# lim0606/pytorch-ardae-vae

Hardware: AMD Instinct MI355X
Metric: AR-DAE-VAE train-steps/sec (batch 512, nz_cdae 256) on dbMNIST (higher is better)
Workload: dtype f32

## Files before the change

### include/ardae_hip.h

```cpp
#ifndef ARDAE_HIP_H
#define ARDAE_HIP_H

#include <stddef.h>
#include <stdint.h>

#ifdef __cplusplus
extern "C" {
#endif

#define ARDAE_ABI_VERSION 1

enum { ARDAE_ACT_NONE = 0, ARDAE_ACT_RELU = 1, ARDAE_ACT_SOFTPLUS = 2, ARDAE_ACT_ELU = 3, ARDAE_ACT_TANH = 4, ARDAE_ACT_LEAKY_RELU = 5, ARDAE_ACT_SWISH = 6 };

enum {
  ARDAE_EPI_ACT = 0,
  ARDAE_EPI_DACT = 1,
  ARDAE_EPI_CHAIN = 2,
  ARDAE_EPI_DAE_LOSS = 3
};

typedef struct ardae_lin_src {
  const float* x;
  int ld;
  int K;
// ... 15 lines not shown
  const float* R; int ldR;
  const float* Q; int ldQ;
  const float* sigma;
  const float* eps; int ldeps;
  float scale;
  float* Y;  int ldY;
  float* Y2; int ldY2;
  float* colsum;
  float* tile_loss;
} ardae_linear_args;

const char* ardae_last_error(void);
int ardae_abi_version(void);

size_t ardae_packed_floats(int nout, int k);
int ardae_linear_row_tiles(int M, int nout);
int ardae_linear_col_panels(int M, int nout);
int ardae_pack_weight(const float* W, int ldw, int nout, int k, int transpose, float* out, void* stream);
int ardae_linear(const ardae_linear_args* args, int epilogue, void* stream);
int ardae_linear_chain_eligible(const ardae_linear_args* layers, int nl, int epilogue);
int ardae_linear_chain(const ardae_linear_args* layers, int nl, int epilogue, void* stream);
int ardae_linear_wide_layers_eligible(const ardae_linear_args* layers, int nl, int epilogue);
int ardae_linear_wide_layers(const ardae_linear_args* layers, int nl, int epilogue, void* stream);


#define ARDAE_WGRAD_MAX_PROBLEMS 20
typedef struct ardae_wgrad_problem {
  int M, O, I;
  int npairs;
  const float* G[2]; int ldG[2];
  const float* X[2]; int ldX[2];
  int bias_pair;
  const float* rowscale;
  int splits;
  float* partial;
  float* partial_vec;
  float* out; int ldout;
  float* out_bias;
  float* out_rowscale; int ld_rowscale;
  float beta;
} ardae_wgrad_problem;
int ardae_wgrad_splits(int M, int O, int I, int nproblems_hint);
int ardae_wgrad_batch(const ardae_wgrad_problem* problems, int nproblems, void* stream);


int ardae_latent_perturb(const float* latent, const float* z0, const float* xi, const float* eps, int B, int nz, int z,
// ... 133 lines not shown
```

### pytorch-ardae-vae_amd/_lib.py

```python
import ctypes
import os

_HERE = os.path.dirname(os.path.abspath(__file__))
LIB_PATH = os.environ.get("ARDAE_LIB") or os.path.join(_HERE, "libardae_hip.so")

c_float_p = ctypes.POINTER(ctypes.c_float)


def debug_knob(name, default=None):
    if os.environ.get("ARDAE_DEBUG_KNOBS") != "1":
        return default
    return os.environ.get(name, default)


class LinSrc(ctypes.Structure):
    _fields_ = [("x", ctypes.c_void_p), ("ld", ctypes.c_int), ("K", ctypes.c_int), ("wp", ctypes.c_void_p)]


class LinearArgs(ctypes.Structure):
    _fields_ = [
        ("M", ctypes.c_int), ("Nout", ctypes.c_int),
        ("nsrc", ctypes.c_int),
        ("src", LinSrc * 2),
        ("act", ctypes.c_int),
# ... 49 lines not shown
MODEL_HEAD_SHIFT = 1
MODEL_CLIPPED = 16
LOGVAR_CLIP = {None: 0, "none": 0, "hard": 1, "softplus": 2, "spm10": 3, "spm6": 4, "spm5": 5, "spm4": 6, "spm3": 7, "spm2": 8, "tanh": 9, "2tanh": 10}
MODEL_CLIP_Z0_SHIFT, MODEL_CLIP_Z_SHIFT = 8, 12


ACT = {"none": 0, None: 0, "relu": 1, "softplus": 2, "csoftplus": 2, "elu": 3, "tanh": 4, "leaky_relu": 5, "swish": 6}
LOG_RECORD_FLOATS = 16
EPI_ACT, EPI_DACT, EPI_CHAIN, EPI_DAE_LOSS = 0, 1, 2, 3

EXPORTS = {
    "ardae_last_error": (ctypes.c_char_p, []),
    "ardae_abi_version": (ctypes.c_int, []),
    "ardae_packed_floats": (ctypes.c_size_t, [ctypes.c_int, ctypes.c_int]),
    "ardae_linear_row_tiles": (ctypes.c_int, [ctypes.c_int, ctypes.c_int]),
    "ardae_linear_col_panels": (ctypes.c_int, [ctypes.c_int, ctypes.c_int]),
    "ardae_pack_weight": (ctypes.c_int, [ctypes.c_void_p, ctypes.c_int, ctypes.c_int, ctypes.c_int, ctypes.c_int,
                                         ctypes.c_void_p, ctypes.c_void_p]),
    "ardae_linear": (ctypes.c_int, [ctypes.POINTER(LinearArgs), ctypes.c_int, ctypes.c_void_p]),
    "ardae_linear_chain_eligible": (ctypes.c_int, [ctypes.POINTER(LinearArgs), ctypes.c_int, ctypes.c_int]),
    "ardae_linear_chain": (ctypes.c_int, [ctypes.POINTER(LinearArgs), ctypes.c_int, ctypes.c_int, ctypes.c_void_p]),
    "ardae_linear_wide_layers_eligible": (ctypes.c_int, [ctypes.POINTER(LinearArgs), ctypes.c_int, ctypes.c_int]),
    "ardae_linear_wide_layers": (ctypes.c_int, [ctypes.POINTER(LinearArgs), ctypes.c_int, ctypes.c_int, ctypes.c_void_p]),
    "ardae_wgrad_splits": (ctypes.c_int, [ctypes.c_int] * 4),
    "ardae_wgrad_batch": (ctypes.c_int, [ctypes.POINTER(WgradProblem), ctypes.c_int, ctypes.c_void_p]),
    "ardae_latent_perturb": (ctypes.c_int, [ctypes.c_void_p] * 4 + [ctypes.c_int] * 3 + [ctypes.c_float] * 2 + [ctypes.c_void_p] * 4),
    "ardae_latent_perturb_nstd": (ctypes.c_int, [ctypes.c_void_p] * 4 + [ctypes.c_int] * 4 + [ctypes.c_float] * 2 + [ctypes.c_void_p] * 4),
    "ardae_latent_perturb_draw_ok": (ctypes.c_int, [ctypes.c_int] * 3),
    "ardae_latent_perturb_draw": (ctypes.c_int, [ctypes.c_void_p] * 2 + [ctypes.c_int] * 3 + [ctypes.c_float] * 2 + [ctypes.c_uint64] * 3 +
                                  [ctypes.c_void_p, ctypes.c_uint64] + [ctypes.c_void_p] * 5),
    "ardae_cdae_perturb_fused_ok": (ctypes.c_int, [ctypes.c_void_p, ctypes.c_int, ctypes.c_int]),
    "ardae_cdae_perturb_loss_grads": (ctypes.c_int, [ctypes.c_void_p] * 6 + [ctypes.c_int] * 2 + [ctypes.c_float] * 2 + [ctypes.c_uint64] * 3 +
                                      [ctypes.c_void_p, ctypes.c_uint64] + [ctypes.c_void_p] * 5 + [ctypes.c_size_t] + [ctypes.c_void_p] * 3),
    "ardae_center_scale": (ctypes.c_int, [ctypes.c_void_p] * 2 + [ctypes.c_int] * 3 + [ctypes.c_float] + [ctypes.c_void_p] * 2),
    "ardae_philox_normal": (ctypes.c_int, [ctypes.c_void_p, ctypes.c_int64, ctypes.c_uint64, ctypes.c_uint64, ctypes.c_void_p]),
    "ardae_philox_uniform": (ctypes.c_int, [ctypes.c_void_p, ctypes.c_int64, ctypes.c_uint64, ctypes.c_uint64, ctypes.c_void_p]),
    "ardae_bernoulli": (ctypes.c_int, [ctypes.c_void_p, ctypes.c_int64, ctypes.c_int, ctypes.c_void_p, ctypes.c_uint64,
                                       ctypes.c_uint64, ctypes.c_void_p]),
    "ardae_step_state_advance": (ctypes.c_int, [ctypes.c_void_p, ctypes.c_uint64, ctypes.c_double, ctypes.c_double, ctypes.c_double, ctypes.c_void_p]),
    "ardae_philox_normal_dev": (ctypes.c_int, [ctypes.c_void_p, ctypes.c_int64, ctypes.c_uint64, ctypes.c_void_p, ctypes.c_uint64, ctypes.c_void_p]),
    "ardae_philox_normal_at": (ctypes.c_int, [ctypes.c_void_p, ctypes.c_int64, ctypes.c_uint64, ctypes.c_uint64, ctypes.c_void_p, ctypes.c_uint64,
                                               ctypes.c_void_p]),
    "ardae_adam_ref_step_dev": (ctypes.c_int, [ctypes.c_void_p] * 5 + [ctypes.c_int64] + [ctypes.c_double] * 3 + [ctypes.c_void_p, ctypes.c_void_p]),
    "ardae_adam_ref_step": (ctypes.c_int, [ctypes.c_void_p] * 5 + [ctypes.c_int64] + [ctypes.c_double] * 4 + [ctypes.c_int, ctypes.c_void_p]),
    "ardae_weight_avg": (ctypes.c_int, [ctypes.c_void_p] * 2 + [ctypes.c_int64, ctypes.c_int, ctypes.c_double, ctypes.c_int64, ctypes.c_void_p,
                                         ctypes.c_int64, ctypes.c_void_p]),
# ... 102 lines not shown
```

### pytorch-ardae-vae_amd/csrc/api.hip

```cpp
#include <stdarg.h>

#include "ardae_hip.h"
#include "common.h"
#include "elementwise.h"
#include "linear.h"
#include "wgrad.h"

namespace ardae {
static thread_local char g_last_error[512] = "";
void set_last_error(const char* fmt, ...) {
  va_list ap;
  va_start(ap, fmt);
  vsnprintf(g_last_error, sizeof(g_last_error), fmt, ap);
  va_end(ap);
}
}

using namespace ardae;

extern "C" {

const char* ardae_last_error(void) { return g_last_error; }
int ardae_abi_version(void) { return ARDAE_ABI_VERSION; }

size_t ardae_packed_floats(int nout, int k) { return packed_floats(nout, k); }
int ardae_linear_row_tiles(int M, int nout) { return linear_row_tiles(M, nout); }
int ardae_linear_col_panels(int M, int nout) { return linear_col_panels(M, nout); }

int ardae_pack_weight(const float* W, int ldw, int nout, int k, int transpose, float* out, void* stream) {
  return launch_pack_weight(W, ldw, nout, k, transpose != 0, out, (hipStream_t)stream);
}

int ardae_linear(const ardae_linear_args* args, int epilogue, void* stream) {
  ARDAE_CHECK_ARG(args != nullptr, "ardae_linear: args is NULL");
  return launch_linear(*args, epilogue, (hipStream_t)stream);
}

int ardae_linear_wide_layers_eligible(const ardae_linear_args* layers, int nl, int epilogue) {
  return layers && linear_wide_layers_eligible(layers, nl, epilogue) ? 1 : 0;
}
int ardae_linear_wide_layers(const ardae_linear_args* layers, int nl, int epilogue, void* stream) {
  ARDAE_CHECK_ARG(layers != nullptr, "ardae_linear_wide_layers: layers is NULL");
  return launch_linear_wide_layers(layers, nl, epilogue, (hipStream_t)stream);
}
int ardae_linear_chain_eligible(const ardae_linear_args* layers, int nl, int epilogue) {
  return (layers != nullptr && linear_chain_eligible(layers, nl, epilogue)) ? 1 : 0;
}
int ardae_linear_chain(const ardae_linear_args* layers, int nl, int epilogue, void* stream) {
  ARDAE_CHECK_ARG(layers != nullptr, "ardae_linear_chain: layers is NULL");
  return launch_linear_chain(layers, nl, epilogue, (hipStream_t)stream);
}

int ardae_wgrad_splits(int M, int O, int I, int nproblems_hint) { return wgrad_splits(M, O, I, nproblems_hint); }
int ardae_wgrad_batch(const ardae_wgrad_problem* problems, int nproblems, void* stream) {
  return launch_wgrad_batch(problems, nproblems, (hipStream_t)stream);
}

int ardae_latent_perturb(const float* latent, const float* z0, const float* xi, const float* eps, int B, int nz, int z,
                         float std_scale, float delta, float* xbar, float* sigma, float* std_b, void* stream) {
  return launch_latent_perturb(latent, z0, xi, eps, B, nz, 1, z, std_scale, delta, xbar, sigma, std_b, (hipStream_t)stream);
}
int ardae_latent_perturb_nstd(const float* latent, const float* z0, const float* xi, const float* eps, int B, int nz, int nstd, int z,
                              float std_scale, float delta, float* xbar, float* sigma, float* std_b, void* stream) {
  return launch_latent_perturb(latent, z0, xi, eps, B, nz, nstd, z, std_scale, delta, xbar, sigma, std_b, (hipStream_t)stream);
}
int ardae_latent_perturb_draw_ok(int nz, int nstd, int z) { return latent_perturb_draw_ok(nz, nstd, z) ? 1 : 0; }
// ... 49 lines not shown
```

### pytorch-ardae-vae_amd/csrc/cdae.hip

```cpp
#include <vector>

#include "ardae_hip.h"
#include "common.h"
#include "elementwise.h"
#include "linear.h"
#include "wgrad.h"

namespace ardae {
namespace {

#define PACK_PUSH(W_, ldw_, nout_, k_, tr_, out_) pack_items__.push_back(PackItem{W_, ldw_, nout_, k_, (tr_) ? 1 : 0, out_})
#define PACK_FLUSH(st_) ARDAE_TRY(launch_pack_batch(pack_items__.data(), (int)pack_items__.size(), st_))

struct Lin {
  size_t w, b;
  int out, in;
};

struct CdaeLayout {
  int kind, z, c, h, L, act;
  std::vector<Lin> ctx, inp, neg;
  size_t total = 0;
  int out_dim() const { return kind == 0 ? 1 : z; }

// ... 118 lines not shown
    PACK_PUSH(params + P.neg[l].w, P.h, P.h, P.h, false, packed + K.neg_f[l]);
    PACK_PUSH(params + P.neg[l].w, P.h, P.h, P.h, true, packed + K.neg_b[l]);
  }
  if (P.kind == 1) {
    PACK_PUSH(params + P.neg[P.L].w, P.h, P.z, P.h, false, packed + K.fc_f);
    PACK_PUSH(params + P.neg[P.L].w, P.h, P.h, P.z, true, packed + K.fc_b);
  }
  PACK_FLUSH(st);
  return 0;
}

LinArgs lin_args(int act, int M, int Nout, const float* x, int ldx, int K, const float* wp, LinArgs a) {
  a.M = M; a.Nout = Nout; a.nsrc = 1; a.act = act;
  a.src[0].x = x; a.src[0].ld = ldx; a.src[0].K = K; a.src[0].wp = wp;
  return a;
}
int lin(int epi, int act, int M, int Nout, const float* x, int ldx, int K, const float* wp, LinArgs a, hipStream_t st) {
  return launch_linear(lin_args(act, M, Nout, x, ldx, K, wp, a), epi, st);
}

struct LayerRun {
  int epi;
  hipStream_t st;
  std::vector<LinArgs> v;
  LayerRun(int epi_, hipStream_t st_) : epi(epi_), st(st_) {}
  void add(int act, int M, int Nout, const float* x, int ldx, int K, const float* wp, LinArgs a) { v.push_back(lin_args(act, M, Nout, x, ldx, K, wp, a)); }
  int flush() {
    size_t i = 0;
    while (i < v.size()) {
      size_t n = v.size() - i;
      while (n >= 2 && !linear_chain_eligible(v.data() + i, (int)n, epi)) --n;
      if (n >= 2) {
        ARDAE_TRY(launch_linear_chain(v.data() + i, (int)n, epi, st));
        i += n;
        continue;
      }
      size_t m = std::min<size_t>(v.size() - i, 6);
      while (m >= 2 && !linear_wide_layers_eligible(v.data() + i, (int)m, epi)) --m;
      if (m >= 2) {
        ARDAE_TRY(launch_linear_wide_layers(v.data() + i, (int)m, epi, st));
        i += m;
      } else {
        ARDAE_TRY(launch_linear(v[i], epi, st));
        i += 1;
      }
    }
    v.clear();
    return 0;
  }
};

float* cdae_a1_slot(const CdaeLayout& P, int B, float* workspace) {
  Bump ws(workspace, ~size_t(0));
  for (int l = 0; l <= P.L; ++l) ws.take((size_t)B * P.h);
  return ws.take(1);
}

int cdae_impl(const ardae_cdae_desc* d, const float* params, const float* packed, const float* xbar, const float* sigma,
              const float* eps, const float* ctx, int B, int S, float* workspace, size_t ws_floats, float* loss, float* grads,
              float* score_out, bool need_grads, hipStream_t st, bool a1_ready = false) {
  ARDAE_TRY(desc_ok(d));
  ARDAE_CHECK_ARG(params && packed && xbar && sigma && ctx && workspace, "cdae: null pointer argument");
  ARDAE_CHECK_ARG(B > 0 && S > 0 && (int64_t)B * S < (int64_t)1 << 30, "cdae: bad batch (B=%d, S=%d)", B, S);
  ARDAE_CHECK_ARG(!need_grads || (eps && loss && grads), "cdae: loss/grads/eps must be given");
  ARDAE_CHECK_ARG(need_grads || score_out, "cdae: score_out is NULL");
  const CdaeLayout P(*d);
  const PackedLayout K(P);
  const int N = B * S, h = P.h, L = P.L, z = P.z, act = P.act;
  ARDAE_CHECK_ARG(ws_floats >= workspace_floats(P, B, S, need_grads), "cdae: workspace too small (%zu < %zu floats)", ws_floats,
                  workspace_floats(P, B, S, need_grads));
// ... 22 lines not shown
    std::vector<LinArgs> pr; std::vector<int> ep, lv;
    int level = 0;
    auto add = [&](const LinArgs& A, int epi, int lev) { pr.push_back(A); ep.push_back(epi); lv.push_back(lev); };
    for (int l = 1; l <= L; ++l, ++level) { add(ctx_layer(l), EPI_ACT, level); add(inp_layer(l), EPI_ACT, level); }
    { LinArgs A{}; A.bias = params + P.neg[0].b; A.Y = cb; A.ldY = h; add(lin_args(ACT_NONE, B, h, cL[L], h, h, packed + K.w1c_f, A), EPI_ACT, level++); }
    for (int l = 1; l <= L; ++l) {
      LinArgs A{}; A.Y = hh[l]; A.ldY = h;
      if (l == 1) { A.rowbias = cb; A.rowbias_ld = h; A.rows_per_group = S; A.rowscale = sigma; A.rowscale_w = W1s; } else A.bias = params + P.neg[l - 1].b;
      if (l == L) { A.Y2 = e[L]; A.ldY2 = h; A.R = wfc0; }
      add(lin_args(act, N, h, l == 1 ? a[L] : hh[l - 1], h, h, l == 1 ? packed + K.w1a_f : packed + K.neg_f[l - 1], A), EPI_ACT, level++);
    }
    for (int l = L; l >= 2; --l) { LinArgs A{}; A.S = hh[l - 1]; A.ldS = h; A.Y = e[l - 1]; A.ldY = h; add(lin_args(act, N, h, e[l], h, h, packed + K.neg_b[l - 1], A), EPI_DACT, level++); }
    { LinArgs A{}; A.S = a[L]; A.ldS = h; A.Y = r[L]; A.ldY = h; add(lin_args(act, N, h, e[1], h, h, packed + K.w1a_b, A), EPI_DACT, level++); }
    for (int l = L; l >= 2; --l) { LinArgs A{}; A.S = a[l - 1]; A.ldS = h; A.Y = r[l - 1]; A.ldY = h; add(lin_args(act, N, h, r[l], h, h, packed + K.inp_b[l - 1], A), EPI_DACT, level++); }
    { LinArgs A{}; A.Y = g; A.ldY = z; add(lin_args(ACT_NONE, N, z, r[1], h, h, packed + K.inp_b[0], A), EPI_ACT, level++); }
    return launch_linear_small_chain(pr.data(), ep.data(), lv.data(), (int)pr.size(), chain_cnt, st);
  }
  ARDAE_CHECK_ARG(!a1_ready || a[1] == cdae_a1_slot(P, B, workspace), "cdae: a_1 slot moved (workspace layout and cdae_a1_slot disagree)");
  const bool few_rows = !a1_ready && linear_small_eligible(inp_layer(1), EPI_ACT);
  auto ctx_bias = [&]() {
    LinArgs A{}; A.bias = params + P.neg[0].b; A.Y = cb; A.ldY = h;
    return lin(EPI_ACT, ACT_NONE, B, h, cL[L], h, h, packed + K.w1c_f, A, st);
  };
  LayerRun run(EPI_ACT, st);
  if (few_rows) {
    for (int l = 1; l <= L; ++l) ARDAE_TRY(launch_linear_pair(ctx_layer(l), inp_layer(l), EPI_ACT, st));
    ARDAE_TRY(ctx_bias());
  } else {
    for (int l = 1; l <= L; ++l) ARDAE_TRY(launch_linear(ctx_layer(l), EPI_ACT, st));
    ARDAE_TRY(ctx_bias());
    for (int l = a1_ready ? 2 : 1; l <= L; ++l) run.v.push_back(inp_layer(l));
  }
  const float* wfc = params + P.neg[L].w;
  {
    for (int l = 1; l <= L; ++l) {
      LinArgs A{}; A.Y = hh[l]; A.ldY = h;
      if (l == 1) {
        A.rowbias = cb; A.rowbias_ld = h; A.rows_per_group = S; A.rowscale = sigma; A.rowscale_w = W1s;
      } else {
        A.bias = params + P.neg[l - 1].b;
      }
      if (P.kind == 0 && l == L) { A.Y2 = e[L]; A.ldY2 = h; A.R = wfc; }
      run.add(act, N, h, l == 1 ? a[L] : hh[l - 1], h, h, l == 1 ? packed + K.w1a_f : packed + K.neg_f[l - 1], A);
    }
    ARDAE_TRY(run.flush());
  }
  const float inv_nz = 1.0f / ((float)N * (float)z);
  if (P.kind == 0) {
    {
      LayerRun run(EPI_DACT, st);
      for (int l = L; l >= 2; --l) {
        LinArgs A{}; A.S = hh[l - 1]; A.ldS = h; A.Y = e[l - 1]; A.ldY = h;
        run.add(act, N, h, e[l], h, h, packed + K.neg_b[l - 1], A);
      }
      {
        LinArgs A{}; A.S = a[L]; A.ldS = h; A.Y = r[L]; A.ldY = h;
        run.add(act, N, h, e[1], h, h, packed + K.w1a_b, A);
      }
      for (int l = L; l >= 2; --l) {
        LinArgs A{}; A.S = a[l - 1]; A.ldS = h; A.Y = r[l - 1]; A.ldY = h;
        run.add(act, N, h, r[l], h, h, packed + K.inp_b[l - 1], A);
      }
      ARDAE_TRY(run.flush());
    }
    if (!need_grads) {
      LinArgs A{}; A.Y = g; A.ldY = z;
      return lin(EPI_ACT, ACT_NONE, N, z, r[1], h, h, packed + K.inp_b[0], A, st);
    }
    LinArgs A{}; A.sigma = sigma; A.eps = eps; A.ldeps = z; A.scale = inv_nz; A.Y = g; A.ldY = z; A.Y2 = gbar; A.ldY2 = z;
    A.tile_loss = tile_loss;
    ARDAE_TRY(lin(EPI_DAE_LOSS, ACT_NONE, N, z, r[1], h, h, packed + K.inp_b[0], A, st));
  } else {
    if (!need_grads) {
      LinArgs A{}; A.bias = params + P.neg[L].b; A.Y = g; A.ldY = z;
      return lin(EPI_ACT, ACT_NONE, N, z, hh[L], h, h, packed + K.fc_f, A, st);
    }
    LinArgs A{}; A.bias = params + P.neg[L].b; A.sigma = sigma; A.eps = eps; A.ldeps = z; A.scale = inv_nz; A.Y = g; A.ldY = z;
    A.Y2 = gbar; A.ldY2 = z; A.tile_loss = tile_loss;
    ARDAE_TRY(lin(EPI_DAE_LOSS, ACT_NONE, N, z, hh[L], h, h, packed + K.fc_f, A, st));
  }
  ARDAE_TRY(launch_sum_scale(tile_loss, ltiles, inv_nz, loss, st));

  float* Qsum = ws.take(Bh);
  for (int l = 1; l <= L; ++l) chat[l] = ws.take(Bh);
  const int ctiles = linear_row_tiles(N, h);
  float* cs_taup = ws.take((size_t)ctiles * h);
  std::vector<float*>&qhat = qbar, &phat = pbar;
  if (P.kind == 0) {
    {
      LayerRun run(EPI_CHAIN, st);
      for (int l = 1; l <= L; ++l) {
        LinArgs A{}; A.S = a[l]; A.ldS = h; A.R = r[l]; A.ldR = h; A.Y = tau[l]; A.ldY = h; A.Y2 = pbar[l]; A.ldY2 = h;
        if (l == 1) run.add(act, N, h, gbar, z, z, packed + K.inp_f[0], A);
        else run.add(act, N, h, tau[l - 1], h, h, packed + K.inp_f[l - 1], A);
      }
      for (int l = 1; l <= L; ++l) {
        LinArgs A{}; A.S = hh[l]; A.ldS = h; A.R = e[l]; A.ldR = h; A.Y = taup[l]; A.ldY = h; A.Y2 = qbar[l]; A.ldY2 = h;
        if (l == L) A.colsum = cs_taup;
        run.add(act, N, h, l == 1 ? tau[L] : taup[l - 1], h, h, l == 1 ? packed + K.w1a_f : packed + K.neg_f[l - 1], A);
      }
      ARDAE_TRY(run.flush());
    }
    ARDAE_TRY(launch_segment_sum(cs_taup, h, 1, ctiles, h, -1.0f, grads + P.neg[L].w, h, st));
    {
      LayerRun run(EPI_DACT, st);
      for (int l = L; l >= 2; --l) {
        LinArgs A{}; A.S = hh[l - 1]; A.ldS = h; A.Q = qbar[l - 1]; A.ldQ = h; A.Y = qhat[l - 1]; A.ldY = h;
        run.add(act, N, h, qhat[l], h, h, packed + K.neg_b[l - 1], A);
      }
      {
        LinArgs A{}; A.S = a[L]; A.ldS = h; A.Q = pbar[L]; A.ldQ = h; A.Y = phat[L]; A.ldY = h;
        run.add(act, N, h, qhat[1], h, h, packed + K.w1a_b, A);
      }
      for (int l = L; l >= 2; --l) {
        LinArgs A{}; A.S = a[l - 1]; A.ldS = h; A.Q = pbar[l - 1]; A.ldQ = h; A.Y = phat[l - 1]; A.ldY = h;
        run.add(act, N, h, phat[l], h, h, packed + K.inp_b[l - 1], A);
      }
      ARDAE_TRY(run.flush());
    }
  } else {
    {
      LinArgs A{}; A.S = hh[L]; A.ldS = h; A.Y = qhat[L]; A.ldY = h;
      ARDAE_TRY(lin(EPI_DACT, act, N, h, gbar, z, z, packed + K.fc_b, A, st));
    }
    for (int l = L; l >= 2; --l) {
      LinArgs A{}; A.S = hh[l - 1]; A.ldS = h; A.Y = qhat[l - 1]; A.ldY = h;
      ARDAE_TRY(lin(EPI_DACT, act, N, h, qhat[l], h, h, packed + K.neg_b[l - 1], A, st));
    }
    {
      LinArgs A{}; A.S = a[L]; A.ldS = h; A.Y = phat[L]; A.ldY = h;
      ARDAE_TRY(lin(EPI_DACT, act, N, h, qhat[1], h, h, packed + K.w1a_b, A, st));
    }
    for (int l = L; l >= 2; --l) {
      LinArgs A{}; A.S = a[l - 1]; A.ldS = h; A.Y = phat[l - 1]; A.ldY = h;
      ARDAE_TRY(lin(EPI_DACT, act, N, h, phat[l], h, h, packed + K.inp_b[l - 1], A, st));
    }
  }
  ARDAE_TRY(launch_segment_sum(qhat[1], h, B, S, h, 1.0f, Qsum, h, st));
  {
    LinArgs A{}; A.S = cL[L]; A.ldS = h; A.Y = chat[L]; A.ldY = h;
    ARDAE_TRY(lin(EPI_DACT, act, B, h, Qsum, h, h, packed + K.w1c_b, A, st));
  }
// ... 110 lines not shown
```

### pytorch-ardae-vae_amd/csrc/linear.h

```cpp
#pragma once
#include "ardae_hip.h"
#include "common.h"

namespace ardae {

using LinSrc = ardae_lin_src;
using LinArgs = ardae_linear_args;

enum Epi : int {
  EPI_ACT = ARDAE_EPI_ACT,
  EPI_DACT = ARDAE_EPI_DACT,
  EPI_CHAIN = ARDAE_EPI_CHAIN,
  EPI_DAE_LOSS = ARDAE_EPI_DAE_LOSS
};

size_t packed_floats(int nout, int k);
int linear_row_tile(int M, int nout);
int linear_row_tiles(int M, int nout);
int linear_col_panels(int M, int nout);

int launch_pack_weight(const float* W, int ldw, int nout, int k, bool transpose, float* out, hipStream_t st);
int launch_linear(const LinArgs& a, int epi, hipStream_t st);
struct PackItem { const float* W; int ldw, nout, k, transpose; float* out; };
constexpr int PACK_BATCH_MAX = 48;
int launch_pack_batch(const PackItem* items, int n, hipStream_t st);
bool linear_small_eligible(const LinArgs& a, int epi);
int launch_linear_small(const LinArgs& a, int epi, hipStream_t st);
int launch_linear_pair(const LinArgs& a0, const LinArgs& a1, int epi, hipStream_t st);
bool linear_wide_layers_eligible(const LinArgs* L, int nl, int epi);
int launch_linear_wide_layers(const LinArgs* L, int nl, int epi, hipStream_t st);
constexpr int LINEAR_SMALL_CHAIN_COUNTER_WORDS = 32;
int launch_linear_small_chain(const LinArgs* probs, const int* epis, const int* level_of, int nprob, float* counters, hipStream_t st);
bool linear_narrow_eligible(const LinArgs& a, int epi);
int launch_linear_narrow(const LinArgs& a, int epi, hipStream_t st);
bool linear_shortk_eligible(const LinArgs& a, int epi);
int launch_linear_shortk(const LinArgs& a, int epi, hipStream_t st);
bool sampler_tail_eligible(const LinArgs& first, int n2);
int launch_sampler_tail(const LinArgs& first, const float* wp2, const float* bias2, float* Z, int ldz, int n2, hipStream_t st,
                        const float* wp2b = nullptr, const float* bias2b = nullptr, float* Zb = nullptr, int ldzb = 0);
bool linear_wide_eligible(const LinArgs& a, int epi);
int launch_linear_wide(const LinArgs& a, int epi, hipStream_t st);

bool linear_chain_eligible(const LinArgs* layers, int nl, int epi);
int launch_linear_chain(const LinArgs* layers, int nl, int epi, hipStream_t st);

}
```

### pytorch-ardae-vae_amd/csrc/linear_wide.hip

```cpp
#include <string.h>

#include "linear_wide_kernel.h"

namespace ardae {
namespace wide {

int wide_grid(int ntiles, int ncp) {
  static const char* genv = debug_knob("ARDAE_WIDE_GRID");
  int g = genv ? atoi(genv) : 256;
  g -= g % ncp;
  return ntiles < g ? ntiles : g;
}

}

namespace {

using namespace wide;

bool al16w(const void* p) { return (reinterpret_cast<uintptr_t>(p) & 15) == 0; }

int wide_panels(const LinArgs& a, int& nch, int& nj) {
  if (a.nsrc != 1) return 0;
  if (a.src[0].K == 256) { nch = 8; nj = 2; return 4; }
// ... 71 lines not shown
    const LinArgs& a = L[l];
    if (!linear_wide_eligible(a, epi)) return false;
    if (a.M != f.M || a.Nout != 256 || a.nsrc != 1 || a.src[0].K != 256 || a.act != f.act || !a.Y) return false;
    if (l > 0 && (a.src[0].x != L[l - 1].Y || a.src[0].ld != L[l - 1].ldY)) return false;
    if (epi == EPI_ACT && (a.rowbias || a.rowscale || a.Y2)) return false;
    if (epi == EPI_DACT && ((a.Q != nullptr) != (f.Q != nullptr))) return false;
    if (epi == EPI_CHAIN && (!a.Y2 || !a.R)) return false;
  }
  return true;
}

int launch_linear_wide_layers(const LinArgs* L, int nl, int epi, hipStream_t st) {
  ARDAE_CHECK_ARG(linear_wide_layers_eligible(L, nl, epi), "linear_wide_layers: run not eligible");
  const int act = L[0].act;
  if (epi == EPI_ACT) return act == ACT_SOFTPLUS ? launch_wide_layers<8, 4, 2, EPI_ACT, ACT_SOFTPLUS, false, false>(L, nl, st)
                                                 : launch_wide_layers<8, 4, 2, EPI_ACT, ACT_RELU, false, false>(L, nl, st);
  if (epi == EPI_CHAIN) return launch_wide_layers<8, 4, 2, EPI_CHAIN, ACT_SOFTPLUS, false, false>(L, nl, st);
  if (L[0].Q) return act == ACT_SOFTPLUS ? launch_wide_layers<8, 4, 2, EPI_DACT, ACT_SOFTPLUS, true, false>(L, nl, st)
                                         : launch_wide_layers<8, 4, 2, EPI_DACT, ACT_RELU, true, false>(L, nl, st);
  return act == ACT_SOFTPLUS ? launch_wide_layers<8, 4, 2, EPI_DACT, ACT_SOFTPLUS, false, false>(L, nl, st)
                             : launch_wide_layers<8, 4, 2, EPI_DACT, ACT_RELU, false, false>(L, nl, st);
}

int launch_linear_wide(const LinArgs& a, int epi, hipStream_t st) {
  switch (epi) {
    case EPI_ACT:
      if (a.act == ACT_NONE) return launch_wide_flags<EPI_ACT, ACT_NONE>(a, st);
      if (a.act == ACT_RELU) return launch_wide_flags<EPI_ACT, ACT_RELU>(a, st);
      if (a.act == ACT_SOFTPLUS) return launch_wide_flags<EPI_ACT, ACT_SOFTPLUS>(a, st);
      break;
    case EPI_DACT:
      if (a.act == ACT_NONE) return launch_wide_flags<EPI_DACT, ACT_NONE>(a, st);
      if (a.act == ACT_RELU) return launch_wide_flags<EPI_DACT, ACT_RELU>(a, st);
      if (a.act == ACT_SOFTPLUS) return launch_wide_flags<EPI_DACT, ACT_SOFTPLUS>(a, st);
      break;
    case EPI_CHAIN:
      if (a.act == ACT_SOFTPLUS) return launch_wide_flags<EPI_CHAIN, ACT_SOFTPLUS>(a, st);
      break;
  }
  ARDAE_CHECK_ARG(false, "linear_wide: unsupported epilogue/activation combination (epi=%d act=%d)", epi, a.act);
  return -1;
}

}
```

### pytorch-ardae-vae_amd/csrc/linear_wide_kernel.h

```cpp
#pragma once
#include <stdlib.h>

#include <algorithm>
#include <type_traits>

#include "linear.h"
#include "profile.h"

#define ARDAE_NT_LD " nt"
#define ARDAE_NT_ST " nt"
namespace ardae {
namespace wide {

constexpr int WBM = 64;
constexpr int WLDW = 68;
constexpr int WBUF_BYTES = WBM * WLDW * 4;
constexpr int NBUF = 3;

typedef __attribute__((address_space(3))) float lds_f32;

template <int OFF>
__device__ __forceinline__ void gload4(f32x4& dst, unsigned voff, const float* sbase) {
  asm volatile("s_nop 4\n\tglobal_load_dwordx4 %0, %1, %2 offset:%3" : "=v"(dst) : "v"(voff), "s"(sbase), "n"(OFF) : "memory");
}
// ... 398 lines not shown
    ChunkOps<6, P, NCH, NP, HP, FT, EPI_T>::run(acc, A, Bw, xv, l0, l1, rb, x);
    ChunkOps<7, P, NCH, NP, HP, FT, EPI_T>::run(acc, A, Bw, xv, l0, l1, rb, x);
  }
}

template <int P, int NCH, int NP, bool HP, bool FT, class EPI_T, class PX>
__device__ __forceinline__ void tile_panels(f32x16 (&acc)[2][EPI_T::NJ], f32x4 (&A)[2][2], f32x4 (&Bw)[wide_slots(NCH, NP, EPI_T::NJ)][EPI_T::NJ], f32x4 (&xv)[PanelGeo<NCH>::NX], f32x2* l0,
                                            f32x2* l1, float (&rb)[EPI_T::NJ], const EPI_T& epi, const i32x4& rX, unsigned xvoff, unsigned xstep, int& buf,
                                            unsigned rlane, unsigned wlane, int row0, int colw, int prev_row0, int tile, int tnext, const PX& panel_x,
                                            const float* wslab, unsigned bvoff, int kch) {
  if constexpr (P < NP) {
    constexpr bool lastp = P + 1 == NP;
    const int bnext = buf + 1 == NBUF ? 0 : buf + 1;
    const PanelCtx<NCH, EPI_T> x{epi, rX, xvoff, xstep, panel_x(lastp ? tnext : tile, lastp ? 0 : P + 1), rlane + buf * WBUF_BYTES, rlane + bnext * WBUF_BYTES,
                                 wlane + bnext * WBUF_BYTES, row0, colw, prev_row0, wslab, bvoff, kch};
    panel<P, NCH, NP, HP, FT>(acc, A, Bw, xv, l0, l1, rb, x);
    buf = bnext;
    tile_panels<P + 1, NCH, NP, HP, FT>(acc, A, Bw, xv, l0, l1, rb, epi, rX, xvoff, xstep, buf, rlane, wlane, row0, colw, prev_row0, tile, tnext, panel_x, wslab,
                                        bvoff, kch);
  }
}

template <int NCH, int NP, int NJ, int EPI, int ACT, bool F1, bool F2>
__device__ __forceinline__ void wide_body(const LinArgs& a, int nrt, int ncp, int tpg) {
  using PG = PanelGeo<NCH>;
  using EPI_T = WideEpi<EPI, ACT, F1, F2, NJ>;
  using SC = Sched<NCH, NP, NJ, EPI_T::NLT, EPI_T::NST, true>;
  constexpr int NX = PG::NX, G = NP * NCH;
  static_assert(NCH % 2 == 0 && NCH >= 4, "fragment double buffer / XW, BAR chunks");
  constexpr int SLOTS = wide_slots(NCH, NP, NJ);
  static_assert(NJ * SLOTS * 4 <= 256 && G % SLOTS == 0, "the slab window must fit the AGPR file");
  __shared__ float lds[NBUF * WBM * WLDW];

#ifdef ARDAE_STAMPS
  const unsigned long long r_kernel = __builtin_amdgcn_s_memrealtime();
#endif
  const int tid = threadIdx.x, lane = tid & 63;
  const int wave = __builtin_amdgcn_readfirstlane(tid >> 6);
  const int l31 = lane & 31, hh = lane >> 5;

  const unsigned lds0 = (unsigned)(uintptr_t)(lds_f32*)lds;
  const unsigned rlane = lds0 + (unsigned)((l31 * WLDW + hh * 4) * 4);
  const unsigned wlane = lds0 + (unsigned)(((tid / PG::C4) * WLDW + (tid % PG::C4) * 4) * 4);

  const int b = (int)blockIdx.x, nwg = (int)gridDim.x;
  const bool xcd_map = ncp > 1 && nwg % (8 * ncp) == 0;
  const int cp = xcd_map ? (b >> 3) % ncp : b % ncp;
  const int rt0 = xcd_map ? ((b >> 3) / ncp) * 8 + (b & 7) : b / ncp;
  const int rts = nwg / ncp;
  const int colw = (cp * 4 * NJ + wave * NJ) * 32;
  EPI_T epi(a, lane);
  epi.column_operands(colw, lane);

  const unsigned ldx4 = (unsigned)a.src[0].ld * 4u;
  const i32x4 rX = make_rsrc(a.src[0].x, (unsigned)a.M * ldx4);
// ... 61 lines not shown
                 : "memory");
    epi.template run<0, !SC::DEFER>(acc, l0, l1, rb, lane, row0, colw, tr);
    if (SC::DEFER) prev_row0 = row0;
#ifdef ARDAE_STAMPS
    t_e += __builtin_amdgcn_s_memtime() - T1;
#endif
  };
  do_tile(std::true_type{});
  for (tile += rts; tile < nrt; tile += rts) do_tile(std::false_type{});
  if (SC::DEFER && prev_row0 >= 0) epi.store_all(l0, l1, prev_row0, colw);
  asm volatile("s_waitcnt vmcnt(0) lgkmcnt(0)" ::: "memory");
#ifdef ARDAE_STAMPS
  if (a.tile_loss != nullptr && lane == 0) {
    unsigned long long* o = reinterpret_cast<unsigned long long*>(a.tile_loss) + ((size_t)blockIdx.x * 4 + wave) * 8;
    const unsigned long long r_end = __builtin_amdgcn_s_memrealtime();
    o[0] = t_k; o[1] = t_e; o[2] = __builtin_amdgcn_s_memtime() - t_begin; o[3] = r_end - r_begin;
    o[4] = r_begin; o[5] = r_end; o[6] = r_kernel;
  }
#endif
}

template <int NCH, int NP, int NJ, int EPI, int ACT, bool F1, bool F2>
__global__ __launch_bounds__(256, 1) void linear_wide_kernel(const LinArgs a, int nrt, int ncp, int tpg) {
  wide_body<NCH, NP, NJ, EPI, ACT, F1, F2>(a, nrt, ncp, tpg);
}

constexpr int WIDE_MAXL = 6;
struct WideLayers {
  int nl;
  LinArgs L[WIDE_MAXL];
};
template <int NCH, int NP, int NJ, int EPI, int ACT, bool F1, bool F2>
__global__ __launch_bounds__(256, 1) void linear_wide_layers_kernel(const WideLayers c, int nrt, int ncp, int tpg) {
  for (int l = 0; l < c.nl; ++l) {
    wide_body<NCH, NP, NJ, EPI, ACT, F1, F2>(c.L[l], nrt, ncp, tpg);
    __syncthreads();
  }
}

int wide_grid(int ntiles, int ncp);

template <int NCH, int NP, int NJ, int EPI, int ACT, bool F1, bool F2>
int launch_wide(const LinArgs& a, hipStream_t st) {
  const int ncp = a.Nout / (128 * NJ);
  const int tpg = (EPI == EPI_ACT && a.rowbias && a.rows_per_group % WBM) ? (a.rows_per_group + WBM - 1) / WBM : 0;
  const int nrt = tpg ? (a.M / a.rows_per_group) * tpg : a.M / WBM;
  const int ntiles = nrt * ncp;
  const int grid = wide_grid(ntiles, ncp);
  if (g_prof_enabled) {
    char name[96];
    snprintf(name, sizeof(name), "linear_wide_kernel<%d, %d, %d, %d, %d, %s, %s>", NCH, NP, NJ, EPI, ACT, F1 ? "true" : "false", F2 ? "true" : "false");
    double ksum = 0;
    for (int s = 0; s < a.nsrc; ++s) ksum += a.src[s].K;
    double tensors = 1.0 + (a.Y2 ? 1 : 0) + ((EPI == EPI_DACT || EPI == EPI_CHAIN) ? 1 : 0) + ((EPI == EPI_CHAIN) ? 1 : 0) +
                     ((EPI == EPI_DACT && a.Q) ? 1 : 0);
    prof_begin(st, name, 2.0 * a.M * (double)a.Nout * ksum, 4.0 * ((double)a.M * ksum + tensors * a.M * (double)a.Nout + ksum * a.Nout));
  }
  hipLaunchKernelGGL((linear_wide_kernel<NCH, NP, NJ, EPI, ACT, F1, F2>), dim3(grid), dim3(256), 0, st, a, nrt, ncp, tpg);
// ... 10 lines not shown
  const int nrt = a.M / WBM;
  const int grid = wide_grid(nrt * ncp, ncp);
  WideLayers c;
  memset(&c, 0, sizeof(c));
  c.nl = nl;
  for (int l = 0; l < nl; ++l) c.L[l] = L[l];
  if (g_prof_enabled) {
    char name[112];
    snprintf(name, sizeof(name), "linear_wide_layers_kernel<%d, %d, %d, %d, %d, %s, %s> x%d", NCH, NP, NJ, EPI, ACT, F1 ? "true" : "false", F2 ? "true" : "false", nl);
    double fl = 0, by = 0;
    for (int l = 0; l < nl; ++l) {
      const double K = L[l].src[0].K;
      const double tensors = 1.0 + (L[l].Y2 ? 1 : 0) + ((EPI == EPI_DACT || EPI == EPI_CHAIN) ? 1 : 0) + ((EPI == EPI_CHAIN) ? 1 : 0) + ((EPI == EPI_DACT && L[l].Q) ? 1 : 0);
      fl += 2.0 * a.M * (double)a.Nout * K;
      by += 4.0 * ((double)a.M * K + tensors * a.M * (double)a.Nout + K * a.Nout);
    }
    prof_begin(st, name, fl, by);
  }
  hipLaunchKernelGGL((linear_wide_layers_kernel<NCH, NP, NJ, EPI, ACT, F1, F2>), dim3(grid), dim3(256), 0, st, c, nrt, ncp, 0);
  prof_end(st);
  ARDAE_LAUNCH_CHECK();
  return 0;
}

#define ARDAE_WIDE_LAYERS_FOR(X)                          \
  X(8, 4, 2, EPI_ACT, ACT_SOFTPLUS, false, false)         \
  X(8, 4, 2, EPI_ACT, ACT_RELU, false, false)             \
  X(8, 4, 2, EPI_DACT, ACT_SOFTPLUS, false, false)        \
  X(8, 4, 2, EPI_DACT, ACT_SOFTPLUS, true, false)         \
  X(8, 4, 2, EPI_DACT, ACT_RELU, false, false)            \
  X(8, 4, 2, EPI_DACT, ACT_RELU, true, false)             \
  X(8, 4, 2, EPI_CHAIN, ACT_SOFTPLUS, false, false)
#define ARDAE_WIDE_LAYERS_EXTERN(NCH, NP, NJ, EPI, ACT, F1, F2) extern template int launch_wide_layers<NCH, NP, NJ, EPI, ACT, F1, F2>(const LinArgs*, int, hipStream_t);
#define ARDAE_WIDE_LAYERS_INSTANTIATE(NCH, NP, NJ, EPI, ACT, F1, F2) template int launch_wide_layers<NCH, NP, NJ, EPI, ACT, F1, F2>(const LinArgs*, int, hipStream_t);
#ifndef ARDAE_WIDE_INST_TU
ARDAE_WIDE_LAYERS_FOR(ARDAE_WIDE_LAYERS_EXTERN)
#endif

#define ARDAE_WIDE_FOR_GEOS(X, EPI, ACT, F1, F2) \
  X(8, 4, 2, EPI, ACT, F1, F2)                    \
  X(4, 1, 2, EPI, ACT, F1, F2)                    \
  X(8, 8, 1, EPI, ACT, F1, F2)
#define ARDAE_WIDE_FOR_ACT_FLAGS(X, ACT)          \
  ARDAE_WIDE_FOR_GEOS(X, EPI_ACT, ACT, false, false) \
  ARDAE_WIDE_FOR_GEOS(X, EPI_ACT, ACT, false, true)  \
  ARDAE_WIDE_FOR_GEOS(X, EPI_ACT, ACT, true, false)  \
// ... 24 lines not shown
```

Baseline: 222.6.

## Fuse mixed-epilogue wide layer runs into one persistent kernel launch

Adds a wide-run kernel that executes up to 12 consecutive 256x256 softplus layers with different epilogues (act, act+Y2, dact, chain, dact+Q), dispatching per layer on a runtime kind and separated by block barriers. The CDAE forward/backward LayerRuns now collect act and dact (or chain and dact) layers into one mixed run, and the segment-sum launch moves after the combined flush. The goal is to remove kernel launch overhead and inter-kernel gaps between epilogue groups. In exchange, the run kernel carries a large argument struct, has more code-size and register pressure from multiple inlined bodies, and loses chain-kernel fusion where that would otherwise apply.

```diff
diff --git a/include/ardae_hip.h b/include/ardae_hip.h
--- a/include/ardae_hip.h
+++ b/include/ardae_hip.h
@@ -61,6 +61,8 @@
 int ardae_linear_chain(const ardae_linear_args* layers, int nl, int epilogue, void* stream);
 int ardae_linear_wide_layers_eligible(const ardae_linear_args* layers, int nl, int epilogue);
 int ardae_linear_wide_layers(const ardae_linear_args* layers, int nl, int epilogue, void* stream);
+int ardae_linear_wide_run_eligible(const ardae_linear_args* layers, const int* epilogues, int nl);
+int ardae_linear_wide_run(const ardae_linear_args* layers, const int* epilogues, int nl, void* stream);
 
 
 #define ARDAE_WGRAD_MAX_PROBLEMS 20
diff --git a/pytorch-ardae-vae_amd/_lib.py b/pytorch-ardae-vae_amd/_lib.py
--- a/pytorch-ardae-vae_amd/_lib.py
+++ b/pytorch-ardae-vae_amd/_lib.py
@@ -95,6 +95,8 @@
     "ardae_linear_chain": (ctypes.c_int, [ctypes.POINTER(LinearArgs), ctypes.c_int, ctypes.c_int, ctypes.c_void_p]),
     "ardae_linear_wide_layers_eligible": (ctypes.c_int, [ctypes.POINTER(LinearArgs), ctypes.c_int, ctypes.c_int]),
     "ardae_linear_wide_layers": (ctypes.c_int, [ctypes.POINTER(LinearArgs), ctypes.c_int, ctypes.c_int, ctypes.c_void_p]),
+    "ardae_linear_wide_run_eligible": (ctypes.c_int, [ctypes.POINTER(LinearArgs), ctypes.POINTER(ctypes.c_int), ctypes.c_int]),
+    "ardae_linear_wide_run": (ctypes.c_int, [ctypes.POINTER(LinearArgs), ctypes.POINTER(ctypes.c_int), ctypes.c_int, ctypes.c_void_p]),
     "ardae_wgrad_splits": (ctypes.c_int, [ctypes.c_int] * 4),
     "ardae_wgrad_batch": (ctypes.c_int, [ctypes.POINTER(WgradProblem), ctypes.c_int, ctypes.c_void_p]),
     "ardae_latent_perturb": (ctypes.c_int, [ctypes.c_void_p] * 4 + [ctypes.c_int] * 3 + [ctypes.c_float] * 2 + [ctypes.c_void_p] * 4),
diff --git a/pytorch-ardae-vae_amd/csrc/api.hip b/pytorch-ardae-vae_amd/csrc/api.hip
--- a/pytorch-ardae-vae_amd/csrc/api.hip
+++ b/pytorch-ardae-vae_amd/csrc/api.hip
@@ -42,6 +42,13 @@
 int ardae_linear_wide_layers(const ardae_linear_args* layers, int nl, int epilogue, void* stream) {
   ARDAE_CHECK_ARG(layers != nullptr, "ardae_linear_wide_layers: layers is NULL");
   return launch_linear_wide_layers(layers, nl, epilogue, (hipStream_t)stream);
+}
+int ardae_linear_wide_run_eligible(const ardae_linear_args* layers, const int* epilogues, int nl) {
+  return linear_wide_run_eligible(layers, epilogues, nl) ? 1 : 0;
+}
+int ardae_linear_wide_run(const ardae_linear_args* layers, const int* epilogues, int nl, void* stream) {
+  ARDAE_CHECK_ARG(layers != nullptr && epilogues != nullptr, "ardae_linear_wide_run: layers / epilogues is NULL");
+  return launch_linear_wide_run(layers, epilogues, nl, (hipStream_t)stream);
 }
 int ardae_linear_chain_eligible(const ardae_linear_args* layers, int nl, int epilogue) {
   return (layers != nullptr && linear_chain_eligible(layers, nl, epilogue)) ? 1 : 0;
diff --git a/pytorch-ardae-vae_amd/csrc/cdae.hip b/pytorch-ardae-vae_amd/csrc/cdae.hip
--- a/pytorch-ardae-vae_amd/csrc/cdae.hip
+++ b/pytorch-ardae-vae_amd/csrc/cdae.hip
@@ -164,30 +164,50 @@
 struct LayerRun {
   int epi;
   hipStream_t st;
+  bool mixed;
   std::vector<LinArgs> v;
-  LayerRun(int epi_, hipStream_t st_) : epi(epi_), st(st_) {}
-  void add(int act, int M, int Nout, const float* x, int ldx, int K, const float* wp, LinArgs a) { v.push_back(lin_args(act, M, Nout, x, ldx, K, wp, a)); }
+  std::vector<int> e;
+  LayerRun(int epi_, hipStream_t st_, bool mixed_ = false) : epi(epi_), st(st_), mixed(mixed_) {}
+  void push(const LinArgs& a) { v.push_back(a); e.push_back(epi); }
+  void add(int act, int M, int Nout, const float* x, int ldx, int K, const float* wp, LinArgs a) { push(lin_args(act, M, Nout, x, ldx, K, wp, a)); }
+  size_t mixed_prefix(size_t i) const {
+    if (!mixed) return 0;
+    size_t m = std::min<size_t>(v.size() - i, LINEAR_WIDE_RUN_MAXL);
+    while (m >= 2 && !linear_wide_run_eligible(v.data() + i, e.data() + i, (int)m)) --m;
+    for (size_t k = i; m >= 2 && k + 1 < i + m; ++k)
+      if (e[k] == e[k + 1] && linear_chain_eligible(v.data() + k, 2, e[k])) return 0;
+    return m >= 2 ? m : 0;
+  }
   int flush() {
     size_t i = 0;
     while (i < v.size()) {
-      size_t n = v.size() - i;
-      while (n >= 2 && !linear_chain_eligible(v.data() + i, (int)n, epi)) --n;
+      if (const size_t m = mixed_prefix(i)) {
+        ARDAE_TRY(launch_linear_wide_run(v.data() + i, e.data() + i, (int)m, st));
+        i += m;
+        continue;
+      }
+      const int ep = e[i];
+      size_t blk = 1;
+      while (i + blk < v.size() && e[i + blk] == ep) ++blk;
+      size_t n = blk;
+      while (n >= 2 && !linear_chain_eligible(v.data() + i, (int)n, ep)) --n;
       if (n >= 2) {
-        ARDAE_TRY(launch_linear_chain(v.data() + i, (int)n, epi, st));
+        ARDAE_TRY(launch_linear_chain(v.data() + i, (int)n, ep, st));
         i += n;
         continue;
       }
-      size_t m = std::min<size_t>(v.size() - i, 6);
-      while (m >= 2 && !linear_wide_layers_eligible(v.data() + i, (int)m, epi)) --m;
+      size_t m = std::min<size_t>(blk, 6);
+      while (m >= 2 && !linear_wide_layers_eligible(v.data() + i, (int)m, ep)) --m;
       if (m >= 2) {
-        ARDAE_TRY(launch_linear_wide_layers(v.data() + i, (int)m, epi, st));
+        ARDAE_TRY(launch_linear_wide_layers(v.data() + i, (int)m, ep, st));
         i += m;
       } else {
-        ARDAE_TRY(launch_linear(v[i], epi, st));
+        ARDAE_TRY(launch_linear(v[i], ep, st));
         i += 1;
       }
     }
     v.clear();
+    e.clear();
     return 0;
   }
 };
@@ -256,14 +276,14 @@
     LinArgs A{}; A.bias = params + P.neg[0].b; A.Y = cb; A.ldY = h;
     return lin(EPI_ACT, ACT_NONE, B, h, cL[L], h, h, packed + K.w1c_f, A, st);
   };
-  LayerRun run(EPI_ACT, st);
+  LayerRun run(EPI_ACT, st, P.kind == 0);
   if (few_rows) {
     for (int l = 1; l <= L; ++l) ARDAE_TRY(launch_linear_pair(ctx_layer(l), inp_layer(l), EPI_ACT, st));
     ARDAE_TRY(ctx_bias());
   } else {
     for (int l = 1; l <= L; ++l) ARDAE_TRY(launch_linear(ctx_layer(l), EPI_ACT, st));
     ARDAE_TRY(ctx_bias());
-    for (int l = a1_ready ? 2 : 1; l <= L; ++l) run.v.push_back(inp_layer(l));
+    for (int l = a1_ready ? 2 : 1; l <= L; ++l) run.push(inp_layer(l));
   }
   const float* wfc = params + P.neg[L].w;
   {
@@ -277,12 +297,12 @@
       if (P.kind == 0 && l == L) { A.Y2 = e[L]; A.ldY2 = h; A.R = wfc; }
       run.add(act, N, h, l == 1 ? a[L] : hh[l - 1], h, h, l == 1 ? packed + K.w1a_f : packed + K.neg_f[l - 1], A);
     }
-    ARDAE_TRY(run.flush());
+    if (P.kind != 0) ARDAE_TRY(run.flush());
   }
   const float inv_nz = 1.0f / ((float)N * (float)z);
   if (P.kind == 0) {
     {
-      LayerRun run(EPI_DACT, st);
+      run.epi = EPI_DACT;
       for (int l = L; l >= 2; --l) {
         LinArgs A{}; A.S = hh[l - 1]; A.ldS = h; A.Y = e[l - 1]; A.ldY = h;
         run.add(act, N, h, e[l], h, h, packed + K.neg_b[l - 1], A);
@@ -322,7 +342,7 @@
   std::vector<float*>&qhat = qbar, &phat = pbar;
   if (P.kind == 0) {
     {
-      LayerRun run(EPI_CHAIN, st);
+      LayerRun run(EPI_CHAIN, st, true);
       for (int l = 1; l <= L; ++l) {
         LinArgs A{}; A.S = a[l]; A.ldS = h; A.R = r[l]; A.ldR = h; A.Y = tau[l]; A.ldY = h; A.Y2 = pbar[l]; A.ldY2 = h;
         if (l == 1) run.add(act, N, h, gbar, z, z, packed + K.inp_f[0], A);
@@ -333,11 +353,7 @@
         if (l == L) A.colsum = cs_taup;
         run.add(act, N, h, l == 1 ? tau[L] : taup[l - 1], h, h, l == 1 ? packed + K.w1a_f : packed + K.neg_f[l - 1], A);
       }
-      ARDAE_TRY(run.flush());
-    }
-    ARDAE_TRY(launch_segment_sum(cs_taup, h, 1, ctiles, h, -1.0f, grads + P.neg[L].w, h, st));
-    {
-      LayerRun run(EPI_DACT, st);
+      run.epi = EPI_DACT;
       for (int l = L; l >= 2; --l) {
         LinArgs A{}; A.S = hh[l - 1]; A.ldS = h; A.Q = qbar[l - 1]; A.ldQ = h; A.Y = qhat[l - 1]; A.ldY = h;
         run.add(act, N, h, qhat[l], h, h, packed + K.neg_b[l - 1], A);
@@ -352,6 +368,7 @@
       }
       ARDAE_TRY(run.flush());
     }
+    ARDAE_TRY(launch_segment_sum(cs_taup, h, 1, ctiles, h, -1.0f, grads + P.neg[L].w, h, st));
   } else {
     {
       LinArgs A{}; A.S = hh[L]; A.ldS = h; A.Y = qhat[L]; A.ldY = h;
diff --git a/pytorch-ardae-vae_amd/csrc/linear.h b/pytorch-ardae-vae_amd/csrc/linear.h
--- a/pytorch-ardae-vae_amd/csrc/linear.h
+++ b/pytorch-ardae-vae_amd/csrc/linear.h
@@ -29,6 +29,9 @@
 int launch_linear_pair(const LinArgs& a0, const LinArgs& a1, int epi, hipStream_t st);
 bool linear_wide_layers_eligible(const LinArgs* L, int nl, int epi);
 int launch_linear_wide_layers(const LinArgs* L, int nl, int epi, hipStream_t st);
+constexpr int LINEAR_WIDE_RUN_MAXL = 12;
+bool linear_wide_run_eligible(const LinArgs* L, const int* epis, int nl);
+int launch_linear_wide_run(const LinArgs* L, const int* epis, int nl, hipStream_t st);
 constexpr int LINEAR_SMALL_CHAIN_COUNTER_WORDS = 32;
 int launch_linear_small_chain(const LinArgs* probs, const int* epis, const int* level_of, int nprob, float* counters, hipStream_t st);
 bool linear_narrow_eligible(const LinArgs& a, int epi);
diff --git a/pytorch-ardae-vae_amd/csrc/linear_wide.hip b/pytorch-ardae-vae_amd/csrc/linear_wide.hip
--- a/pytorch-ardae-vae_amd/csrc/linear_wide.hip
+++ b/pytorch-ardae-vae_amd/csrc/linear_wide.hip
@@ -117,6 +117,49 @@
                              : launch_wide_layers<8, 4, 2, EPI_DACT, ACT_RELU, false, false>(L, nl, st);
 }
 
+namespace {
+int wide_kind(const LinArgs& a, int epi) {
+  if (epi == EPI_ACT) return a.Y2 ? (a.rowscale ? -1 : WK_ACT_Y2) : a.rowscale ? WK_ACT_RS : WK_ACT;
+  if (epi == EPI_DACT) return a.Q ? WK_DACT_Q : WK_DACT;
+  if (epi == EPI_CHAIN) return WK_CHAIN;
+  return -1;
+}
+bool in_set(int k, std::initializer_list<int> set) { return std::find(set.begin(), set.end(), k) != set.end(); }
+const std::initializer_list<int> RUN_FWD = {WK_ACT, WK_ACT_RS, WK_ACT_Y2, WK_DACT}, RUN_BWD = {WK_CHAIN, WK_DACT_Q};
+}
+
+bool linear_wide_run_eligible(const LinArgs* L, const int* epis, int nl) {
+  static const bool on = !(debug_knob("ARDAE_WIDE_LAYERS") && atoi(debug_knob("ARDAE_WIDE_LAYERS")) == 0);
+  if (!on || !L || !epis || nl < 2 || nl > WIDE_RUN_MAXL) return false;
+  const LinArgs& f = L[0];
+  const bool fwd = in_set(wide_kind(f, epis[0]), RUN_FWD);
+  for (int l = 0; l < nl; ++l) {
+    const LinArgs& a = L[l];
+    const int k = wide_kind(a, epis[l]);
+    if (!in_set(k, fwd ? RUN_FWD : RUN_BWD)) return false;
+    if (!linear_wide_eligible(a, epis[l])) return false;
+    if (a.M != f.M || a.Nout != 256 || a.nsrc != 1 || a.src[0].K != 256 || a.act != ACT_SOFTPLUS || !a.Y) return false;
+    if (l > 0) {
+      const LinArgs& p = L[l - 1];
+      const int pk = wide_kind(p, epis[l - 1]);
+      const bool from_y = a.src[0].x == p.Y && a.src[0].ld == p.ldY;
+      const bool from_y2 = (pk == WK_ACT_Y2 || pk == WK_CHAIN) && p.Y2 && a.src[0].x == p.Y2 && a.src[0].ld == p.ldY2;
+      if (!from_y && !from_y2) return false;
+    }
+    if (a.rowbias && a.rows_per_group % WBM) return false;
+    if (k == WK_CHAIN && (!a.Y2 || !a.R)) return false;
+  }
+  return true;
+}
+
+int launch_linear_wide_run(const LinArgs* L, const int* epis, int nl, hipStream_t st) {
+  ARDAE_CHECK_ARG(linear_wide_run_eligible(L, epis, nl), "linear_wide_run: run not eligible");
+  int kinds[WIDE_RUN_MAXL];
+  for (int l = 0; l < nl; ++l) kinds[l] = wide_kind(L[l], epis[l]);
+  if (in_set(kinds[0], RUN_FWD)) return launch_wide_run<ARDAE_WIDE_RUN_FWD>(L, kinds, nl, st);
+  return launch_wide_run<ARDAE_WIDE_RUN_BWD>(L, kinds, nl, st);
+}
+
 int launch_linear_wide(const LinArgs& a, int epi, hipStream_t st) {
   switch (epi) {
     case EPI_ACT:
diff --git a/pytorch-ardae-vae_amd/csrc/linear_wide_inst_run_bwd.hip b/pytorch-ardae-vae_amd/csrc/linear_wide_inst_run_bwd.hip
--- /dev/null
+++ b/pytorch-ardae-vae_amd/csrc/linear_wide_inst_run_bwd.hip
@@ -0,0 +1,10 @@
+#define ARDAE_WIDE_INST_TU
+#include <string.h>
+
+#include "linear_wide_kernel.h"
+
+namespace ardae {
+namespace wide {
+template int launch_wide_run<ARDAE_WIDE_RUN_BWD>(const LinArgs*, const int*, int, hipStream_t);
+}
+}
diff --git a/pytorch-ardae-vae_amd/csrc/linear_wide_inst_run_fwd.hip b/pytorch-ardae-vae_amd/csrc/linear_wide_inst_run_fwd.hip
--- /dev/null
+++ b/pytorch-ardae-vae_amd/csrc/linear_wide_inst_run_fwd.hip
@@ -0,0 +1,10 @@
+#define ARDAE_WIDE_INST_TU
+#include <string.h>
+
+#include "linear_wide_kernel.h"
+
+namespace ardae {
+namespace wide {
+template int launch_wide_run<ARDAE_WIDE_RUN_FWD>(const LinArgs*, const int*, int, hipStream_t);
+}
+}
diff --git a/pytorch-ardae-vae_amd/csrc/linear_wide_kernel.h b/pytorch-ardae-vae_amd/csrc/linear_wide_kernel.h
--- a/pytorch-ardae-vae_amd/csrc/linear_wide_kernel.h
+++ b/pytorch-ardae-vae_amd/csrc/linear_wide_kernel.h
@@ -444,7 +444,7 @@
 }
 
 template <int NCH, int NP, int NJ, int EPI, int ACT, bool F1, bool F2>
-__device__ __forceinline__ void wide_body(const LinArgs& a, int nrt, int ncp, int tpg) {
+__device__ __forceinline__ void wide_body(const LinArgs& a, int nrt, int ncp, int tpg, float* lds) {
   using PG = PanelGeo<NCH>;
   using EPI_T = WideEpi<EPI, ACT, F1, F2, NJ>;
   using SC = Sched<NCH, NP, NJ, EPI_T::NLT, EPI_T::NST, true>;
@@ -452,7 +452,6 @@
   static_assert(NCH % 2 == 0 && NCH >= 4, "fragment double buffer / XW, BAR chunks");
   constexpr int SLOTS = wide_slots(NCH, NP, NJ);
   static_assert(NJ * SLOTS * 4 <= 256 && G % SLOTS == 0, "the slab window must fit the AGPR file");
-  __shared__ float lds[NBUF * WBM * WLDW];
 
 #ifdef ARDAE_STAMPS
   const unsigned long long r_kernel = __builtin_amdgcn_s_memrealtime();
@@ -560,7 +559,8 @@
 
 template <int NCH, int NP, int NJ, int EPI, int ACT, bool F1, bool F2>
 __global__ __launch_bounds__(256, 1) void linear_wide_kernel(const LinArgs a, int nrt, int ncp, int tpg) {
-  wide_body<NCH, NP, NJ, EPI, ACT, F1, F2>(a, nrt, ncp, tpg);
+  __shared__ float lds[NBUF * WBM * WLDW];
+  wide_body<NCH, NP, NJ, EPI, ACT, F1, F2>(a, nrt, ncp, tpg, lds);
 }
 
 constexpr int WIDE_MAXL = 6;
@@ -570,8 +570,43 @@
 };
 template <int NCH, int NP, int NJ, int EPI, int ACT, bool F1, bool F2>
 __global__ __launch_bounds__(256, 1) void linear_wide_layers_kernel(const WideLayers c, int nrt, int ncp, int tpg) {
+  __shared__ float lds[NBUF * WBM * WLDW];
   for (int l = 0; l < c.nl; ++l) {
-    wide_body<NCH, NP, NJ, EPI, ACT, F1, F2>(c.L[l], nrt, ncp, tpg);
+    wide_body<NCH, NP, NJ, EPI, ACT, F1, F2>(c.L[l], nrt, ncp, tpg, lds);
+    __syncthreads();
+  }
+}
+
+enum WideKind { WK_ACT = 0, WK_ACT_RS = 1, WK_ACT_Y2 = 2, WK_DACT = 3, WK_DACT_Q = 4, WK_CHAIN = 5 };
+constexpr int WIDE_RUN_MAXL = LINEAR_WIDE_RUN_MAXL;
+struct WideRun {
+  int nl;
+  int kind[WIDE_RUN_MAXL];
+  LinArgs L[WIDE_RUN_MAXL];
+};
+static_assert(sizeof(WideRun) <= 4000, "kernel arguments are limited to 4 KiB");
+template <int K> struct KindEpi;
+template <> struct KindEpi<WK_ACT> { static constexpr int EPI = EPI_ACT; static constexpr bool F1 = false, F2 = false; };
+template <> struct KindEpi<WK_ACT_RS> { static constexpr int EPI = EPI_ACT; static constexpr bool F1 = false, F2 = true; };
+template <> struct KindEpi<WK_ACT_Y2> { static constexpr int EPI = EPI_ACT; static constexpr bool F1 = true, F2 = false; };
+template <> struct KindEpi<WK_DACT> { static constexpr int EPI = EPI_DACT; static constexpr bool F1 = false, F2 = false; };
+template <> struct KindEpi<WK_DACT_Q> { static constexpr int EPI = EPI_DACT; static constexpr bool F1 = true, F2 = false; };
+template <> struct KindEpi<WK_CHAIN> { static constexpr int EPI = EPI_CHAIN; static constexpr bool F1 = false, F2 = false; };
+
+template <int ACT, int K0, int... KS>
+__device__ __forceinline__ void wide_run_layer(int kind, const LinArgs& a, int nrt, int ncp, float* lds) {
+  if (kind == K0) {
+    using E = KindEpi<K0>;
+    wide_body<8, 4, 2, E::EPI, ACT, E::F1, E::F2>(a, nrt, ncp, 0, lds);
+  } else if constexpr (sizeof...(KS) > 0) {
+    wide_run_layer<ACT, KS...>(kind, a, nrt, ncp, lds);
+  }
+}
+template <int ACT, int... KS>
+__global__ __launch_bounds__(256, 1) void linear_wide_run_kernel(const WideRun c, int nrt, int ncp) {
+  __shared__ float lds[NBUF * WBM * WLDW];
+  for (int l = 0; l < c.nl; ++l) {
+    wide_run_layer<ACT, KS...>(c.kind[l], c.L[l], nrt, ncp, lds);
     __syncthreads();
   }
 }
@@ -628,6 +663,43 @@
   ARDAE_LAUNCH_CHECK();
   return 0;
 }
+
+template <int ACT, int... KS>
+int launch_wide_run(const LinArgs* L, const int* kinds, int nl, hipStream_t st) {
+  const LinArgs& a = L[0];
+  const int ncp = a.Nout / 256;
+  const int nrt = a.M / WBM;
+  const int grid = wide_grid(nrt * ncp, ncp);
+  WideRun c;
+  memset(&c, 0, sizeof(c));
+  c.nl = nl;
+  for (int l = 0; l < nl; ++l) { c.kind[l] = kinds[l]; c.L[l] = L[l]; }
+  if (g_prof_enabled) {
+    char name[112];
+    int n = snprintf(name, sizeof(name), "linear_wide_run_kernel<%d", ACT);
+    for (int k : {KS...}) n += snprintf(name + n, sizeof(name) - n, ", %d", k);
+    snprintf(name + n, sizeof(name) - n, "> x%d", nl);
+    double fl = 0, by = 0;
+    for (int l = 0; l < nl; ++l) {
+      const int k = kinds[l];
+      const double K = L[l].src[0].K;
+      const double tensors = 1.0 + (L[l].Y2 ? 1 : 0) + (k >= WK_DACT ? 1 : 0) + (k == WK_CHAIN ? 1 : 0) + (k == WK_DACT_Q ? 1 : 0);
+      fl += 2.0 * a.M * (double)a.Nout * K;
+      by += 4.0 * ((double)a.M * K + tensors * a.M * (double)a.Nout + K * a.Nout);
+    }
+    prof_begin(st, name, fl, by);
+  }
+  hipLaunchKernelGGL((linear_wide_run_kernel<ACT, KS...>), dim3(grid), dim3(256), 0, st, c, nrt, ncp);
+  prof_end(st);
+  ARDAE_LAUNCH_CHECK();
+  return 0;
+}
+#define ARDAE_WIDE_RUN_FWD ACT_SOFTPLUS, WK_ACT, WK_ACT_RS, WK_ACT_Y2, WK_DACT
+#define ARDAE_WIDE_RUN_BWD ACT_SOFTPLUS, WK_CHAIN, WK_DACT_Q
+#ifndef ARDAE_WIDE_INST_TU
+extern template int launch_wide_run<ARDAE_WIDE_RUN_FWD>(const LinArgs*, const int*, int, hipStream_t);
+extern template int launch_wide_run<ARDAE_WIDE_RUN_BWD>(const LinArgs*, const int*, int, hipStream_t);
+#endif
 
 #define ARDAE_WIDE_LAYERS_FOR(X)                          \
   X(8, 4, 2, EPI_ACT, ACT_SOFTPLUS, false, false)         \
```

Result: no change. 223.2, median of 6 (+0.3%).
